# HazyResearch/sampler

Measured on AMD Instinct MI355X. Metric: variables sampled/sec (whole node), higher is better.
Workload: dtype f64 (f32 sampling weights)

## Files before the change

sampler_amd/csrc/dwx_api.cc:

```cpp
#include "../../include/dwx.h"

#include <algorithm>
#include <array>
#include <chrono>
#include <cstdio>
#include <cstdlib>
#include <cmath>
#include <cstring>
#include <map>
#include <memory>
#include <new>
#include <stdexcept>
#include <string>
#include <vector>

#include "device_build.h"
#include "graph_compile.h"
#include "host_parallel.h"
#include "level_build.h"
#if defined(DWX_EMU) && !defined(DWX_EMU_LEVEL_BUILD_UNIT)
#include "level_build.cc"
#endif

#include "sweep_kernels.h"
// ... 64 lines not shown
template <class T>
T *upload_raw(const T *h, size_t n, rt::stream_t s) {
  T *d = (T *)rt::dmalloc(n * sizeof(T));
  rt::h2d(d, h, n * sizeof(T), s);
  return d;
}

struct TimedSpan {
  rt::event_t a, b, c;
  int kind;
  uint32_t launches;
  bool has_pull;
  bool new_sweep;
  uint32_t n_sweeps = 1;
};

template <class... A>
struct Variant {
  void (*fn)(A...) = nullptr;
  size_t lds = 0;
  unsigned cap = 1;
  bool allowed = false;
  void allow() {
    if (!allowed) { rt::allow_dynamic_lds(fn, lds); allowed = true; }
  }
  static Variant eager(void (*f)(A...), size_t bytes) {
    Variant v;
    v.fn = f; v.lds = bytes;
    v.allow();
    v.cap = rt::resident_blocks(f, BLOCK_THREADS, bytes);
    return v;
  }
  Variant lazy(void (*f)(A...)) const {
    Variant v = *this;
    v.fn = f; v.allowed = false;
    return v;
  }
  template <class... B>
  void launch(unsigned grid, unsigned block, rt::stream_t st, B... args) {
    if (!fn) throw std::logic_error("a sweep kernel build that dwx_sampler_create did not resolve for this graph");
    allow();
    rt::launch(fn, grid, block, lds, st, args...);
  }
};
using SweepVariant = Variant<KernelParams>;
using SortedVariant = Variant<KernelParams, const SuperTile *, uint32_t, const SortRec8 *, const double *, uint32_t>;
struct SweepVariants {
  SweepVariant infer[2];
  SweepVariant learn, learn_pull;
  SweepVariant tab[2];
  SweepVariant multi[2][2];
  Variant<KernelParams, MergeArgs> merged[2];
  Variant<KernelParams, PersistArgs> persist;
  SortedVariant sorted_infer[2][2], sorted_learn[2];
};
}

struct dwx_graph {
  std::shared_ptr<CompiledGraph> cg;
};

struct dwx_sampler {
  std::shared_ptr<CompiledGraph> cg;
  dwx_options opts;
  int device = 0;
  rt::stream_t stream = nullptr;
  rt::stream_t side[2] = {nullptr, nullptr};
  rt::event_t ev_fork = nullptr, ev_join[2] = {nullptr, nullptr};
  uint32_t *d_v_meta = nullptr, *d_v_orig = nullptr, *d_v_row = nullptr, *d_v_init = nullptr;
  uint32_t *d_row_ptr = nullptr;
  TileDesc *d_tiles = nullptr;
  uint32_t *d_giant = nullptr, *d_wide = nullptr;
  std::vector<uint32_t> cgiant_tiles, bgiant_tiles, bgiant_piece_off;
  uint32_t *d_bgiant = nullptr, *d_bgiant_piece_off = nullptr, *d_bgiant_decision = nullptr;
  GiantPiece *d_bgiant_pieces = nullptr;
  double *d_bgiant_partial = nullptr;
  int stage_k = 12;
  struct Chunk { uint32_t launch, t0, t1; };
  std::vector<Chunk> plan_chunks;
  uint32_t plan_batches = 1;
  double plan_eta = 0.0;
  bool plan_valid = false;
  std::map<uint32_t, double> row_sum_cache;
  std::vector<uint64_t> sgd_work;
  uint64_t sgd_work_max_launch = 0;
  bool wide_learn = false;
  bool tv_pair = false;
  SweepVariants kv;
  bool rec8 = false;
  bool rp_cat = false;
  bool all_pull = false;
  EdgeRec8 *d_edges8 = nullptr;
  SortRec8 *d_sorted = nullptr;
  SuperTile *d_supers = nullptr;
  double *d_sort_dvals = nullptr;
  uint32_t n_sort_dvals = 0;
  bool sorted_learn = false;
  bool no_sort_uni = false;
  bool sorted_fallback_said = false;
  double *d_row_truth = nullptr, *d_edge_fval64 = nullptr;
  EdgeRec *d_edges = nullptr;
  VifRec *d_vifs = nullptr;
  uint32_t *d_assign_free = nullptr, *d_assign_evid = nullptr, *d_tally = nullptr;
  double *d_weights = nullptr;
  float *d_w32 = nullptr;
  double *d_w_init = nullptr;
  EdgeTerms *d_terms = nullptr;
  int terms_state = 0;
  unsigned long long *d_rb = nullptr;
  bool rb_on = false;
  unsigned long long *d_trace = nullptr;
  uint32_t trace_cap = 0, trace_words = 0, trace_bits = 0;
  uint32_t trace_next = 0, trace_count = 0;
  bool trace_on = false;
  std::vector<uint64_t> trace_ids;
  FactorRec *d_frecs = nullptr;
  VifRec *d_fvifs = nullptr;
  double *d_ffval64 = nullptr;
  uint32_t *d_fwide = nullptr;
  bool score_ready = false;
  bool wstats_ready = false;
  uint64_t wstats_max_count = 0, wstats_max_wid = 0;
  long long *d_pot = nullptr;
  int pot_alloc = 0;
  std::vector<uint8_t> pot_valid;
  bool pot_wanted = false;
  bool last_infer = false;
  bool pot_query_first = false;
  uint64_t pot_supers = 0, pot_sweeps = 0;
  struct Pending {
    bool owed = false;
    bool evid_owed = false;
    uint64_t sweep = 0;
    bool snap = false;
    std::vector<uint8_t> cached;
  } pending;
  bool defer_ok = false;
  float *d_w32_prev = nullptr;
  uint64_t deferred_sweeps = 0, flushes = 0;
  bool has_simple_tiles = false;
  unsigned long long *d_delta = nullptr;
  struct Level {
    std::vector<Chunk> chunks;
    bool fast = false;
    uint32_t *d_inc_wid = nullptr, *d_inc_slot = nullptr;
    float *d_inc_d = nullptr;
    std::vector<uint32_t> inc_begin, inc_end;
    long long *d_t_static = nullptr;
    uint32_t rows = 0;
    double c_max = 0.0, t_max = 0.0;
    std::string range_error;
// ... 161 lines not shown
    rt::event_record(s->ev_fork, s->stream);
    if (any_giant) rt::stream_wait_event(st_giant, s->ev_fork);
    if (any_wide) rt::stream_wait_event(st_wide, s->ev_fork);
  }
  auto launch_lane_tiles = [&](uint32_t a, uint32_t b) {
  if (b <= a) return;
  P.tile_begin = a;
  P.tile_end = b;
  const bool tab8 = s->rec8 && !LEARN && P.edge_terms;
  const bool slim = LEARN && s->rec8 && s->all_pull && !(P.flags & OPT_NO_PULL);
  SweepVariant &k = multi ? kv.multi[rb][trace] : tab8 ? kv.tab[rb] : !LEARN ? kv.infer[rb] : slim ? kv.learn_pull : kv.learn;
  k.launch(std::min<unsigned>(b - a, k.cap), BLOCK_THREADS, s->stream, P);
  ++launches;
  };
  bool used_sorted = false;
  if (s->d_supers && !P.edge_terms && !multi && (!LEARN || (s->sorted_learn && !(P.flags & (OPT_NO_PULL | OPT_DYNAMIC_T))))) {
    const dwx_sampler::Level *lv =
        (LEARN && !P.pot && !default_layout && s->plan_level && s->plan_level->d_supers) ? s->plan_level : nullptr;
    const std::vector<SuperTile> &sv = lv ? lv->sorted_supers : c.supers;
    const SuperTile *d_sv = lv ? lv->d_supers : s->d_supers;
    const SortRec8 *d_sr = lv ? lv->d_sorted : s->d_sorted;
    size_t a = std::lower_bound(sv.begin(), sv.end(), t0, [](const SuperTile &x, uint32_t t) { return x.tile0 < t; }) - sv.begin();
    size_t b = a;
    while (b < sv.size() && sv[b].tile0 + sv[b].ntiles <= t1) ++b;
    struct Run { size_t a, b; };
    std::vector<Run> runs;
    for (size_t i = a; i < b;) {
      size_t j = i + 1;
      while (j < b && sv[j].tile0 == sv[j - 1].tile0 + sv[j - 1].ntiles) ++j;
      runs.push_back({i, j});
      i = j;
    }
    if (runs.size() > 8 && !s->sorted_fallback_said) {
      s->sorted_fallback_said = true;
      fprintf(stderr, "dwx: a launch's weight-sorted super-tiles form %zu gap-free runs (more than 8): its tiles take "
                      "the plain tile sweep (slower weight gathers)\n", runs.size());
    }
    if (!runs.empty() && runs.size() <= 8) {
      used_sorted = true;
      if (covered && sv[runs[0].a].tile0 == t0) *covered = sv[runs[0].b - 1].tile0 + sv[runs[0].b - 1].ntiles;
      uint32_t cursor = t0;
      for (const Run &r : runs) {
        launch_lane_tiles(cursor, sv[r.a].tile0);
        P.super_rot = 0;
        if (LEARN && P.pot) {
          uint32_t n_cached = 0;
          for (size_t i = r.a; i < r.b; ++i)
            if (sv[i].v0 >= P.pot_v0 && sv[i].v0 + sv[i].nv <= P.pot_v1) ++n_cached;
          s->pot_supers += n_cached;
          if (!s->pot_query_first && n_cached < r.b - r.a && sv[r.a].v0 >= P.pot_v0 && sv[r.a].v0 + sv[r.a].nv <= P.pot_v1)
            P.super_rot = n_cached;
        }
        const bool uni = s->n_sort_dvals == 2 && !s->no_sort_uni;
        (LEARN ? kv.sorted_learn[uni] : kv.sorted_infer[uni][rb])
            .launch((unsigned)(r.b - r.a), SORT_THREADS, s->stream, P, (const SuperTile *)(d_sv + r.a), (uint32_t)(r.b - r.a), d_sr,
                    (const double *)s->d_sort_dvals, s->n_sort_dvals);
        ++launches;
        P.super_rot = 0;
        cursor = sv[r.b - 1].tile0 + sv[r.b - 1].ntiles;
      }
      launch_lane_tiles(cursor, t1);
    }
  }
  if (!used_sorted) launch_lane_tiles(t0, t1);
  P.tile_begin = t0;
  P.tile_end = t1;
  if (cg1 > cg0) {
    rt::launch(rb ? giant_kernel<LEARN, RBK> : giant_kernel<LEARN>, cg1 - cg0, GIANT_THREADS, 0, st_giant, P,
               (const uint32_t *)(s->d_giant + cg0), cg1 - cg0);
    ++launches;
  }
  if (bg1 > bg0) {
    const uint32_t p0 = s->bgiant_piece_off[bg0], np = s->bgiant_piece_off[bg1] - p0;
    rt::launch(giant_pot_kernel<LEARN>, np, GIANT_THREADS, 0, st_giant, P, (const uint32_t *)s->d_bgiant,
               (const GiantPiece *)s->d_bgiant_pieces, p0, np, s->d_bgiant_partial);
    rt::launch(rb ? giant_decide_kernel<LEARN, RBK> : giant_decide_kernel<LEARN>, (bg1 - bg0 + BLOCK_THREADS - 1) / BLOCK_THREADS,
               BLOCK_THREADS, 0, st_giant, P, (const uint32_t *)s->d_bgiant, (const uint32_t *)s->d_bgiant_piece_off, bg0, bg1 - bg0,
               (const double *)s->d_bgiant_partial, s->d_bgiant_decision);
    launches += 2;
    if (LEARN) {
      rt::launch(giant_grad_kernel, np, GIANT_THREADS, 0, st_giant, P, (const uint32_t *)s->d_bgiant,
                 (const GiantPiece *)s->d_bgiant_pieces, p0, np, (const uint32_t *)s->d_bgiant_decision);
      ++launches;
    }
  }
  if (w1 > w0) {
    const uint32_t per_block = BLOCK_THREADS / 64u;
    rt::launch(rb ? wide_kernel<LEARN, RBK> : wide_kernel<LEARN>, (w1 - w0 + per_block - 1) / per_block, BLOCK_THREADS, 0,
               st_wide, P, (const uint32_t *)(s->d_wide + w0), w1 - w0);
    ++launches;
  }
  if (fork) {
    if (any_giant) { rt::event_record(s->ev_join[0], st_giant); rt::stream_wait_event(s->stream, s->ev_join[0]); }
    if (any_wide) { rt::event_record(s->ev_join[1], st_wide); rt::stream_wait_event(s->stream, s->ev_join[1]); }
  }
  return launches;
}

bool multi_sweep_graph(const dwx_sampler *s) {
  return s->rec8 && no_binned_tiles(s) && !getenv("DWX_NO_MULTI_SWEEP");
}

void flush_pending(dwx_sampler *s, int chains = 3);
void trace_pack(dwx_sampler *s, uint64_t first_id, uint32_t n_planes, bool unsampled_only) {
  const CompiledGraph &c = *s->cg;
  if (!unsampled_only) flush_pending(s, 2);
  const uint32_t n = (uint32_t)c.Vo;
// ... 877 lines not shown
      t_phase = t;
    };
    s->d_v_meta = upload(c.v_meta, st, 1);
    s->d_v_orig = upload(c.perm, st, 1);
    s->d_v_row = upload(c.v_row, st);
    s->d_v_init = upload(c.v_init, st, 1);
    s->d_row_ptr = upload(c.row_ptr, st, 1);
    {
      std::vector<TileDesc> tiles = c.tiles;
      if (c.ecap > 6 * BLOCK_THREADS) for (auto &t : tiles) t.flags &= ~(TILE_TERMS2 | TILE_TERMS3 | TILE_PULL_UNARY);
      s->d_tiles = upload(tiles, st);
    }
    for (uint32_t ti : c.giant_tiles) ((c.tiles[ti].flags & TILE_CATEGORICAL) ? s->cgiant_tiles : s->bgiant_tiles).push_back(ti);
    s->d_giant = upload(s->cgiant_tiles, st);
    s->d_wide = upload(c.wide_tiles, st);
    {
      std::vector<GiantPiece> pieces;
      s->bgiant_piece_off.assign(1, 0u);
      for (uint32_t slot = 0; slot < s->bgiant_tiles.size(); ++slot) {
        const TileDesc &td = c.tiles[s->bgiant_tiles[slot]];
        for (uint32_t e = td.e0; e < td.e0 + td.nedges; e += GIANT_PIECE)
          pieces.push_back(GiantPiece{slot, e, std::min(e + GIANT_PIECE, td.e0 + td.nedges), 0u});
        if (!td.nedges) pieces.push_back(GiantPiece{slot, td.e0, td.e0, 0u});
        s->bgiant_piece_off.push_back((uint32_t)pieces.size());
      }
      s->d_bgiant = upload(s->bgiant_tiles, st);
      s->d_bgiant_piece_off = upload(s->bgiant_piece_off, st);
      s->d_bgiant_pieces = upload(pieces, st);
      s->d_bgiant_partial = (double *)rt::dmalloc(std::max<size_t>(1, pieces.size()) * 4 * 8);
      rt::dmemset(s->d_bgiant_partial, 0, std::max<size_t>(1, pieces.size()) * 4 * 8, st);
      s->d_bgiant_decision = (uint32_t *)rt::dmalloc(std::max<size_t>(1, s->bgiant_tiles.size()) * 16);
    }
    if (!c.row_truth.empty()) s->d_row_truth = upload(c.row_truth, st);
    if (!c.edge_fval64.empty()) s->d_edge_fval64 = upload(c.edge_fval64, st);
    s->d_edges = upload(c.edges, st, 1);
    s->rec8 = c.edges8.size() != 0;
    if (s->rec8) s->d_edges8 = upload(c.edges8, st, 1);
    s->defer_ok = s->rec8 && !opts->learn_non_evidence && !opts->noise_aware && !getenv("DWX_NO_DEFER");
    if (!c.supers.empty()) {
      s->d_supers = upload(c.supers, st);
      if (c.sorted_deferred) {
        s->d_sorted = (SortRec8 *)rt::dmalloc((c.n_sorted + 1) * sizeof(SortRec8));
        rt::dmemset(s->d_sorted + c.n_sorted, 0, sizeof(SortRec8), st);
        devb::build_sorted_records(s->d_tiles, s->d_edges, s->d_edges8, s->d_supers, (uint32_t)c.supers.size(),
                                   c.sort_dbits.data(), (uint32_t)c.sort_dbits.size(), c.n_sorted, s->d_sorted, (void *)st);
      } else {
        s->d_sorted = upload(c.sorted_recs, st, 1);
      }
      s->d_sort_dvals = upload(c.sort_dvals, st);
      s->n_sort_dvals = (uint32_t)c.sort_dvals.size();
      s->sorted_learn = c.W > LDS_AGG_MAX_W;
      const size_t lds_sorted = sort_lds_bytes(s->n_sort_dvals);
      auto set = [&](SortedVariant &k, auto fn, bool rb) { k.fn = fn; k.lds = lds_sorted; if (!rb) k.allow(); };
      set(s->kv.sorted_infer[0][0], sorted_sweep_kernel<false, false>, false);
      set(s->kv.sorted_infer[0][1], sorted_sweep_kernel<false, false, true>, true);
      set(s->kv.sorted_infer[1][0], sorted_sweep_kernel<false, true>, false);
      set(s->kv.sorted_infer[1][1], sorted_sweep_kernel<false, true, true>, true);
      set(s->kv.sorted_learn[0], sorted_sweep_kernel<true, false>, false);
      set(s->kv.sorted_learn[1], sorted_sweep_kernel<true, true>, false);
      s->no_sort_uni = getenv("DWX_NO_SORT_UNI") != nullptr;
      s->pot_query_first = getenv("DWX_POT_QUERY_FIRST") != nullptr;
    }
    {
      std::vector<VifRec> vifs = c.vifs;
      if (vifs.size() < 4) vifs.resize(4, VifRec{0u, 0u});
      s->d_vifs = upload(vifs, st, 4);
    }
    std::vector<uint32_t> a0(c.V);
    for (uint64_t p = 0; p < c.V; ++p) a0[p] = (c.v_meta[p] & VM_EVIDENCE) ? c.v_init[p] : 0u;
    s->d_assign_free = upload(a0, st);
    s->d_assign_evid = upload(a0, st);
    s->d_tally = (uint32_t *)rt::dmalloc((c.R + 1) * 4);
    rt::dmemset(s->d_tally, 0, (c.R + 1) * 4, st);
    s->d_weights = upload(c.w_init, st);
    phase("upload graph");
    {
      std::vector<float> w32(c.W);
      for (uint64_t i = 0; i < c.W; ++i) w32[i] = (float)c.w_init[i];
      s->d_w32 = upload(w32, st, 1);
      const size_t n_delta = c.tiles.size() * 8 + 2 + (size_t)BP1_TILES * 8;
      s->d_delta = (unsigned long long *)rt::dmalloc(n_delta * 8);
      rt::dmemset(s->d_delta, 0, n_delta * 8, st);
    }
    s->d_w_fixed = upload(c.w_fixed, st);
    s->d_grad = (long long *)rt::dmalloc(c.W * 16);
    rt::dmemset(s->d_grad, 0, c.W * 16, st);

    KernelParams &P = s->base;
    P.v_meta = s->d_v_meta; P.v_orig = s->d_v_orig; P.v_row = s->d_v_row; P.v_init = s->d_v_init;
    P.row_ptr = s->d_row_ptr; P.row_truth = s->d_row_truth; P.edges = s->d_edges; P.edges8 = s->d_edges8; P.edge_terms = nullptr;
    for (const TileDesc &td : c.tiles) if (td.flags & (TILE_SIMPLE | TILE_INLINE2)) { s->has_simple_tiles = true; break; }
    P.edge_fval64 = s->d_edge_fval64; P.vifs = s->d_vifs; P.tiles = s->d_tiles;
    P.assign_free = s->d_assign_free; P.assign_evid = s->d_assign_evid; P.tally = s->d_tally;
    P.w32 = s->d_w32; P.grad = s->d_grad; P.delta = s->d_delta;
    P.seed = opts->seed; P.sweep = 0; P.vid_offset = opts->var_id_offset; P.tile_begin = 0; P.num_weights = (uint32_t)c.W;
    P.flags = (opts->sample_evidence ? OPT_SAMPLE_EVIDENCE : 0) |
              (opts->learn_non_evidence ? OPT_LEARN_NON_EVIDENCE : 0) |
              (opts->noise_aware ? OPT_NOISE_AWARE : 0) |
              (c.has_f64_fval ? OPT_HAS_F64_FVAL : 0) | (c.has_truthiness ? OPT_HAS_TRUTHINESS : 0);
    P.ecap = c.ecap; P.rcap = c.rcap;
    if (c.ecap > MAX_ECAP) throw std::invalid_argument("tile_edges exceeds the staging capacity");
    s->stage_k = c.ecap <= 3 * BLOCK_THREADS ? 3 : (c.ecap <= 6 * BLOCK_THREADS ? 6 : 12);
    const size_t slots = (size_t)s->stage_k * BLOCK_THREADS;
    s->rp_cat = c.edges8.size() != 0 && c.has_categorical && s->stage_k == 6;
    const size_t nrp = std::max<size_t>(c.rcap + 1, (s->rp_cat ? ROWPTR_UNROLL_CAT : ROWPTR_UNROLL) * BLOCK_THREADS);
    size_t off = (nrp * 4 + 15) & ~(size_t)15;
    P.lds_pot_off = c.has_categorical ? (uint32_t)off : 0u;
    if (c.has_categorical) off += (size_t)c.rcap * 8;
    off = (off + 15) & ~(size_t)15;
    P.lds_edge_off = (uint32_t)off;
    s->wide_learn = c.n_terms2_tiles > 0 && s->stage_k <= 6;
    off += slots * sizeof(EdgeRec);
// ... 1275 lines not shown
```

sampler_amd/csrc/sweep_kernels.h:

```cpp
#ifndef DWX_SWEEP_KERNELS_H_
#define DWX_SWEEP_KERNELS_H_

#include <type_traits>

#include "tile_walk.h"

namespace dwx {

DWX_DEV float rec8_signed(uint32_t code, float f) {
  const uint32_t b = float_to_bits(f);
  return bits_to_float(code == 1u ? 0u : (code == 0u ? (b ^ 0x80000000u) : b));
}
DWX_DEV EdgeRec expand_record(const EdgeRec8 &c) {
  EdgeRec r;
  r.wid = c.key & REC8_WID_MASK;
  r.fval = rec8_signed((c.key >> REC8_HIT_SHIFT) & 3u, c.f);
  r.aux = float_to_bits(rec8_signed((c.key >> REC8_MISS_SHIFT) & 3u, c.f));
  r.packed = EDGE_PRESIGNED | (1u << EDGE_ARITY_SHIFT) | ((c.key & REC8_FIXED) ? EDGE_FIXED_FLAG : 0u);
  return r;
}
DWX_DEV EdgeRec expand_record(const EdgeRec &r) { return r; }

template <int K, class Rec = EdgeRec, int RP = (int)ROWPTR_UNROLL>
struct TilePrefetch {
// ... 466 lines not shown
    TileDesc raw_nn = d;
    if (!ONE) {
      raw_nn = P.tiles[has_nn ? nn : tile];
      TileDesc dl = dn;
      if (!has_next) { dl.nedges = 0; dl.nrows = 0; dl.nv = 1; }
      issue_tile_loads<LEARN, K, !TAB>(P, dl, t, f);
    }
    int delta = 0;
    if (MULTI) {
      if (fits) {
        TileView T{s_rowptr, d.r0, s_edges, d.e0, s_w, s_agg, P.lds_pot_off ? s_pot : nullptr};
        const uint32_t n = P.n_sweeps;
        const uint32_t S = (n >= MULTI_SLICE_MIN_SWEEPS && d.nv < BLOCK_THREADS) ? MULTI_SLICES : 1u;
        if (TRACE && P.trace_bits == 1u) {
          infer_bool_multi_trace<W_TERMS, true, RB>(P, T, d.v0 + t, pre, n, t < d.nv);
        } else if (S == 1u) {
          if (t < d.nv) infer_variable_multi<W_TERMS, true, RB, TRACE>(P, T, d.v0 + t, pre, 0u, n, true);
        } else for (uint32_t item = t; item < S * d.nv; item += BLOCK_THREADS) {
          const uint32_t sl = item / d.nv, var = item - sl * d.nv;
          const VarPre vp = var == t ? pre : load_var_pre<false, false>(P, d.v0 + var);
          const uint32_t k_lo = (uint32_t)((uint64_t)n * sl / S), k_hi = (uint32_t)((uint64_t)n * (sl + 1) / S);
          infer_variable_multi<W_TERMS, true, RB, TRACE>(P, T, d.v0 + var, vp, k_lo, k_hi, sl + 1 == S);
        }
      }
    } else if (fits && t < d.nv) {
      TileView T{s_rowptr, d.r0, s_edges, d.e0, s_w, s_agg, P.lds_pot_off ? s_pot : nullptr};
      if (LEARN && pull)
        delta = process_variable<LEARN, W_TERMS8, true, true>(P, T, d.v0 + t, pre, A, B, true);
      else
        process_variable<LEARN, LEARN ? W_ARRAY : (TAB ? W_TERMS8 : W_TERMS), true, true, false, RB>(P, T, d.v0 + t, pre, A, B, false);
    }
    if (pull) {
      const unsigned long long nz = DWX_BALLOT(delta != 0), ng = DWX_BALLOT(delta < 0);
      if ((t & 63u) == 0) {
        unsigned long long *wd = P.delta + ((size_t)tile * 4 + (t >> 6)) * 2;
        DWX_NT_STORE(nz, &wd[0]); DWX_NT_STORE(ng, &wd[1]);
      }
    }
    if (ONE || !has_next) break;
    __syncthreads();
    d = dn;
    dn = scalarise(raw_nn);
    tile = next; next = nn; has_next = has_nn;
  }
  flush_accumulators(P, s_agg, t);
}
template <bool LEARN, int K, bool TAB = false, int RP = (int)ROWPTR_UNROLL, bool MULTI = false, bool RB = false,
          bool TRACE = false>
__global__ void __launch_bounds__(BLOCK_THREADS, TAB ? 4 : (LEARN ? DWX_S8_LEARN_WG : DWX_S8_INFER_WG)) sweep8_kernel(const KernelParams P) {
  sweep8_body<LEARN, K, TAB, RP, MULTI, false, false, RB, TRACE>(P, nullptr);
}


template <bool LEARN, bool UNI = false, bool RB = false>
__global__ void __launch_bounds__(SORT_THREADS, SORT_WG_PER_CU)
sorted_sweep_kernel(const KernelParams P, const SuperTile *supers, uint32_t n_supers, const SortRec8 *recs,
                    const double *dvals, uint32_t n_dvals) {
  DWX_DYN_LDS(dyn_lds);
  uint32_t *s_tv = (uint32_t *)dyn_lds;
  double *s_d = (double *)(dyn_lds + sort_acc_offset(0));
  unsigned long long *s_acc = (unsigned long long *)(dyn_lds + sort_acc_offset(UNI ? 0u : DWX_UNIFORM(n_dvals)));
  const uint32_t t = threadIdx.x;
  if (blockIdx.x >= n_supers) return;
  const uint32_t b = blockIdx.x + P.super_rot;
  SuperTile S = supers[b < n_supers ? b : b - n_supers];
  S.tile0 = DWX_UNIFORM(S.tile0); S.ntiles = DWX_UNIFORM(S.ntiles); S.v0 = DWX_UNIFORM(S.v0); S.nv = DWX_UNIFORM(S.nv);
  S.lo = DWX_UNIFORM(S.lo); S.hi = DWX_UNIFORM(S.hi); S.nrec = DWX_UNIFORM(S.nrec);
  const bool cached = LEARN && P.pot && S.v0 >= P.pot_v0 && S.v0 + S.nv <= P.pot_v1;
  if (cached) S.nrec = 0;
  const SortRec8 *base = recs + (((uint64_t)S.hi << 32) | S.lo);
  SortRec8 rec[SORT_K];
  DWX_LOAD_SORTED_RECORDS(SORT_K, base, S.nrec, 0u, t, rec);
  const double d_uni = UNI ? dvals[1] : 0.0;
  if (!UNI) for (uint32_t i = t; i < n_dvals; i += SORT_THREADS) s_d[i] = dvals[i];
  for (uint32_t i = t; i < S.ntiles; i += SORT_THREADS) s_tv[i] = P.tiles[S.tile0 + i].v0;
  if (t == 0) s_tv[S.ntiles] = S.v0 + S.nv;
  for (uint32_t i = t; i < S.nv; i += SORT_THREADS) s_acc[i] = 0ull;
  __syncthreads();
  constexpr uint32_t STEP = SORT_K * SORT_THREADS;
  for (uint32_t first = 0; first < S.nrec; first += STEP) {
    float w[SORT_K];
#pragma unroll
    for (int k = 0; k < SORT_K; ++k) w[k] = P.w32[rec[k].wid];
    SortRec8 cur[SORT_K];
#pragma unroll
    for (int k = 0; k < SORT_K; ++k) cur[k] = rec[k];
    DWX_LOAD_SORTED_RECORDS(SORT_K, base, S.nrec, first + STEP, t, rec);
#pragma unroll
    for (int k = 0; k < SORT_K; ++k) {
      const uint32_t di = cur[k].od >> SORT_OWNER_BITS;
      const long long q = pot_fix((double)w[k] * (UNI ? d_uni : s_d[di]));
      if (di) atomicAdd(&s_acc[cur[k].od & SORT_OWNER_MASK], (unsigned long long)q);
    }
  }
  constexpr uint32_t TPB = SORT_THREADS / BLOCK_THREADS;
  const uint32_t lane = t & (BLOCK_THREADS - 1), sub = t / BLOCK_THREADS;
  struct Pass { bool have; uint32_t tile, p; bool live; VarPre pre; long long sum; };
  auto issue = [&](uint32_t j0) {
    Pass ps;
    ps.have = j0 + sub < S.ntiles;
    const uint32_t j = ps.have ? j0 + sub : 0u;
    const uint32_t tv0 = s_tv[j], tnv = s_tv[j + 1] - tv0;
    ps.tile = S.tile0 + j;
    ps.live = ps.have && lane < tnv;
    ps.p = tv0 + (lane < tnv ? lane : tnv - 1u);
    ps.pre = load_var_pre<LEARN>(P, ps.p);
    ps.sum = cached ? DWX_NT_LOAD(&P.pot[ps.p]) : 0ll;
    return ps;
  };
  Pass nxt = issue(0u);
  __syncthreads();
  for (uint32_t j0 = 0; j0 < S.ntiles; j0 += TPB) {
    const Pass ps = nxt;
    nxt = issue(j0 + TPB < S.ntiles ? j0 + TPB : j0);
    int delta = 0;
    if (ps.live) {
      double A, B;
      philox_uniforms(P.seed, P.vid_offset + ps.pre.orig, P.sweep, A, B);
      const long long sum = cached ? ps.sum : (long long)s_acc[ps.p - S.v0];
      if (!LEARN && P.pot) DWX_NT_STORE(sum, &P.pot[ps.p]);
      const double x = pot_unfix(sum);
      TileView T{nullptr, 0u, nullptr, 0u, nullptr, nullptr, nullptr};
      T.presum = &x;
      delta = process_variable<LEARN, W_FIXSUM, true, false, false, RB>(P, T, ps.p, ps.pre, A, B, true);
    }
    if (LEARN) {
      const unsigned long long nz = DWX_BALLOT(delta != 0), ng = DWX_BALLOT(delta < 0);
      if (ps.have && (t & 63u) == 0) {
        unsigned long long *wd = P.delta + ((size_t)ps.tile * 4 + (lane >> 6)) * 2;
        DWX_NT_STORE(nz, &wd[0]); DWX_NT_STORE(ng, &wd[1]);
      }
    }
  }
}

template <bool LEARN, bool RB = false>
__global__ void __launch_bounds__(GIANT_THREADS) giant_kernel(const KernelParams P, const uint32_t *giant_tiles,
                                                              uint32_t n) {
  if (blockIdx.x >= n) return;
  const TileDesc d = P.tiles[giant_tiles[blockIdx.x]];
  const uint32_t p = d.v0;
  const VarPre vp = load_var_pre<LEARN>(P, p);
  double A, B;
  philox_uniforms(P.seed, P.vid_offset + vp.orig, P.sweep, A, B);
  const TileView T{P.row_ptr, 0u, P.edges, 0u, nullptr, nullptr, nullptr};
  process_variable<LEARN, W_COOPB, false, false, false, RB>(P, T, p, vp, A, B);
}

struct GiantPiece { uint32_t slot, e0, e1, pad; };

template <bool LEARN>
__global__ void __launch_bounds__(GIANT_THREADS)
giant_pot_kernel(const KernelParams P, const uint32_t *bgiant_tiles, const GiantPiece *pieces, uint32_t piece0,
                 uint32_t n, double *partial) {
  if (blockIdx.x >= n) return;
  const GiantPiece pc = pieces[piece0 + blockIdx.x];
  const uint32_t p = P.tiles[bgiant_tiles[pc.slot]].v0;
  const TileView T{P.row_ptr, 0u, P.edges, 0u, nullptr, nullptr, nullptr};
  double acc[4] = {0.0, 0.0, 0.0, 0.0};
  if (LEARN) {
    const uint32_t *const chains[2] = {P.assign_free, P.assign_evid};
    const int chain[4] = {0, 0, 1, 1};
    const uint32_t prop[4] = {1u, 0u, 1u, 0u};
    const bool hit[4] = {true, false, true, false};
    coop_for_records<W_COOPB, 4, 2>(P, T, pc.e0, pc.e1, p, chains, chain, prop, hit,
                                    [&](const EdgeRec &, uint32_t, double w, const double (&term)[4]) {
#pragma unroll
                                      for (int j = 0; j < 4; ++j) acc[j] += w * term[j];
                                    });
  } else {
    const uint32_t *const chains[1] = {P.assign_evid};
    const int chain[2] = {0, 0};
    const uint32_t prop[2] = {1u, 0u};
    const bool hit[2] = {true, false};
    coop_for_records<W_COOPB, 2, 1>(P, T, pc.e0, pc.e1, p, chains, chain, prop, hit,
                                    [&](const EdgeRec &, uint32_t, double w, const double (&term)[2]) {
                                      acc[2] += w * term[0];
                                      acc[3] += w * term[1];
                                    });
  }
#pragma unroll
  for (int j = LEARN ? 0 : 2; j < 4; ++j) {
    const double v = block_sum_all(acc[j]);
// ... 58 lines not shown
```

sampler_amd/csrc/tile_walk.h:

```cpp
#ifndef DWX_TILE_WALK_H_
#define DWX_TILE_WALK_H_

#include "factor_functions.h"

namespace dwx {

enum { W_GLOBAL = 0, W_ARRAY = 1, W_INRECORD = 2, W_TERMS = 3, W_TERMS8 = 4, W_COOP = 5, W_COOPB = 6, W_PRESUM = 7, W_LREC = 8, W_FIXSUM = 9 };
#ifndef DWX_GIANT_PIECE
#define DWX_GIANT_PIECE 4096
#endif
constexpr uint32_t GIANT_PIECE = DWX_GIANT_PIECE;
#ifndef DWX_GIANT_THREADS
#define DWX_GIANT_THREADS 1024
#endif
constexpr uint32_t GIANT_THREADS = DWX_GIANT_THREADS;
constexpr uint32_t COOP_U = 4;

DWX_DEV uint32_t wave_lane() { return threadIdx.x & 63u; }

DWX_DEV double block_sum_all(double v) {
  __shared__ double s_red[GIANT_THREADS];
  const uint32_t t = threadIdx.x;
  s_red[t] = v;
  __syncthreads();
// ... 691 lines not shown
  if (WMODE == W_LREC) {
    const LearnRec *recs = (const LearnRec *)T.edges;
    const bool evid_hits = evid_value == hit_value, free_hits = free_value == hit_value;
    for (uint32_t e = es; e < ee; ++e) {
      const LearnRec r = recs[e - T.edge_bias];
      if (r.packed & EDGE_FIXED_FLAG) continue;
      const double g = (double)(free_hits ? r.sf1 : r.sf0) - (double)(evid_hits ? r.se1 : r.se0);
      const long long gi = llrint(FIX_SCALE * (t * g));
      const long long ti = count_t ? llrint(FIX_SCALE * t) : 0;
      long long *dst = T.agg ? T.agg : P.grad;
      if (gi) atomicAdd((unsigned long long *)&dst[r.wid], (unsigned long long)gi);
      if (count_t) atomicAdd((unsigned long long *)&dst[P.num_weights + r.wid], (unsigned long long)ti);
    }
    return;
  }
  for (uint32_t e = es; e < ee; ++e) {
    const EdgeRec er = T.edges[e - T.edge_bias];
    if (er.packed & EDGE_FIXED_FLAG) continue;
    double pot_evid, pot_free;
    if (SIMPLE || (er.packed & EDGE_PRESIGNED)) {
      pot_evid = edge_term<true>(P, er, e, P.assign_evid, me, evid_value, evid_value == hit_value);
      pot_free = edge_term<true>(P, er, e, P.assign_free, me, free_value, free_value == hit_value);
    } else {
      const double fv = (er.packed & EDGE_F64_FLAG) ? P.edge_fval64[e] : (double)er.fval;
      const uint32_t prop[2] = {evid_value, free_value};
      double sg[2];
      if (edge_arity(er) == 1u) {
        sg[0] = unary_sign(edge_func(er), prop[0] == er.aux); sg[1] = unary_sign(edge_func(er), prop[1] == er.aux);
      } else {
        const uint32_t *const chains[2] = {P.assign_evid, P.assign_free};
        const int chain[2] = {0, 1};
        record_signs<2, 2>(P, er, me, chains, chain, prop, sg);
      }
      pot_evid = sg[0] * fv;
      pot_free = sg[1] * fv;
    }
    const double g = pot_free - pot_evid;
    const long long gi = llrint(FIX_SCALE * (t * g));
    const long long ti = count_t ? llrint(FIX_SCALE * t) : 0;
    if (T.agg) {
      if (gi) atomicAdd((unsigned long long *)&T.agg[er.wid], (unsigned long long)gi);
      if (count_t) atomicAdd((unsigned long long *)&T.agg[P.num_weights + er.wid], (unsigned long long)ti);
    } else {
      if (gi) atomicAdd((unsigned long long *)&P.grad[er.wid], (unsigned long long)gi);
      if (count_t) atomicAdd((unsigned long long *)&P.grad[P.num_weights + er.wid], (unsigned long long)ti);
    }
  }
}

struct VarPre {
  uint32_t meta, orig, row0, init;
};

template <bool LEARN, bool NT = true>
DWX_DEV VarPre load_var_pre(const KernelParams &P, uint32_t p) {
  VarPre v;
  if (NT) {
    v.meta = DWX_NT_LOAD(&P.v_meta[p]);
    v.orig = DWX_NT_LOAD(&P.v_orig[p]);
    v.row0 = DWX_NT_LOAD(&P.v_row[p]);
    v.init = LEARN ? DWX_NT_LOAD(&P.v_init[p]) : 0u;
  } else {
    v.meta = P.v_meta[p];
    v.orig = P.v_orig[p];
    v.row0 = P.v_row[p];
    v.init = LEARN ? P.v_init[p] : 0u;
  }
  return v;
}

struct TraceCursor {
  uint32_t slot = 0;
  DWX_DEV void init(const KernelParams &P, uint32_t k_lo) {
    const uint32_t k0 = k_lo > P.trace_skip ? k_lo : P.trace_skip;
    slot = (uint32_t)(((uint64_t)P.trace_slot0 + (k0 - P.trace_skip)) % P.trace_cap);
  }
  DWX_DEV unsigned long long *plane(const KernelParams &P) const { return P.trace + (size_t)slot * P.trace_words; }
  DWX_DEV void next(const KernelParams &P) { if (++slot == P.trace_cap) slot = 0; }
};
DWX_DEV void trace_byte(const KernelParams &P, TraceCursor &c, uint32_t k, uint32_t p, uint32_t value) {
  if (k >= P.trace_skip) {
    ((unsigned char *)c.plane(P))[p] = (unsigned char)value;
    c.next(P);
  }
}
template <int WMODE, bool FIXED, bool RB = false, bool TRACE = false>
DWX_DEV void infer_variable_multi(const KernelParams &P, const TileView &T, uint32_t p, const VarPre pre,
                                  const uint32_t k_lo, const uint32_t k_hi, const bool store) {
  const uint32_t meta = pre.meta;
  if ((meta & VM_EVIDENCE) && !(P.flags & OPT_SAMPLE_EVIDENCE)) return;
  const uint32_t card = meta >> VM_CARD_SHIFT, row0 = pre.row0;
  const uint64_t vid = P.vid_offset + pre.orig;
  uint32_t prop = 0;
  TraceCursor tc;
  if (TRACE) tc.init(P, k_lo);
  if (!(meta & VM_CATEGORICAL)) {
    double pp, pn;
    bool_potentials<WMODE, true, FIXED>(P, T, row0, P.assign_evid, p, pp, pn);
    const double scale = 1.0 + exp(pn - pp);
    uint32_t count = 0;
    for (uint32_t k = k_lo; k < k_hi; ++k) {
      double A, B;
      philox_uniforms(P.seed, vid, P.sweep + k, A, B);
      prop = (A * scale < 1.0) ? 1u : 0u;
      count += prop;
      if (TRACE) trace_byte(P, tc, k, p, prop);
    }
    if (count) atomicAdd(&P.tally[row0], count);
    if (RB && k_hi > k_lo) rb_add(P, row0, (unsigned long long)(k_hi - k_lo) * rb_bool_q(pp, pn));
  } else if (card <= SMALL_CARD) {
// ... 46 lines not shown
#pragma unroll
    for (uint32_t d = 0; d < SMALL_CARD; ++d)
      if (d < card && cnt[d]) atomicAdd(&P.tally[row0 + d], cnt[d]);
  } else {
    for (uint32_t k = k_lo; k < k_hi; ++k) {
      double A, B;
      philox_uniforms(P.seed, vid, P.sweep + k, A, B);
      prop = cat_draw<WMODE, true, RB>(P, T, row0, card, P.assign_evid, p, A);
      atomicAdd(&P.tally[row0 + prop], 1u);
      if (TRACE) trace_byte(P, tc, k, p, prop);
    }
  }
  if (store) DWX_NT_STORE(prop, &P.assign_evid[p]);
}

template <int WMODE, bool FIXED, bool RB>
DWX_DEV void infer_bool_multi_trace(const KernelParams &P, const TileView &T, uint32_t p, const VarPre pre,
                                    const uint32_t n, const bool in_tile) {
  const bool active = in_tile && !((pre.meta & VM_EVIDENCE) && !(P.flags & OPT_SAMPLE_EVIDENCE));
  const uint32_t row0 = pre.row0;
  const uint64_t vid = P.vid_offset + pre.orig;
  double pp = 0.0, pn = 0.0;
  if (active) bool_potentials<WMODE, true, FIXED>(P, T, row0, P.assign_evid, p, pp, pn);
  const double scale = 1.0 + exp(pn - pp);
  const uint32_t lane = threadIdx.x & 63u, p0 = p - lane;
  const uint32_t sh = p0 & 63u;
  const size_t w = p0 >> 6;
  TraceCursor tc;
  tc.init(P, 0u);
  uint32_t prop = 0, count = 0;
  for (uint32_t k = 0; k < n; ++k) {
    if (active) {
      double A, B;
      philox_uniforms(P.seed, vid, P.sweep + k, A, B);
      prop = (A * scale < 1.0) ? 1u : 0u;
      count += prop;
    }
    const unsigned long long m = DWX_BALLOT(active && prop);
    if (k >= P.trace_skip) {
      if (lane == 0 && m) {
        unsigned long long *plane = tc.plane(P);
        atomicAdd(&plane[w], m << sh);
        if (sh && (m >> (64u - sh))) atomicAdd(&plane[w + 1], m >> (64u - sh));
      }
      tc.next(P);
    }
  }
  if (!active) return;
  if (count) atomicAdd(&P.tally[row0], count);
  if (RB && n) rb_add(P, row0, (unsigned long long)n * rb_bool_q(pp, pn));
  DWX_NT_STORE(prop, &P.assign_evid[p]);
}

template <bool LEARN, int WMODE, bool SIMPLE, bool FIXED = false, bool NOCAT = false, bool RB = false>
DWX_DEV int process_variable(const KernelParams &P, const TileView &T, uint32_t p,
                             const VarPre pre, double A, double B, const bool want_delta = false) {
  const uint32_t meta = pre.meta;
  const bool is_cat = !NOCAT && (meta & VM_CATEGORICAL);
  const bool is_evid = meta & VM_EVIDENCE;
  const uint32_t card = meta >> VM_CARD_SHIFT;
  const uint32_t row0 = pre.row0;
  static_assert(!(LEARN && RB), "Rao-Blackwellised sums: inference sweeps only");
  constexpr bool COOP = Coop<WMODE>::on;
  const bool leader = !COOP || Coop<WMODE>::lane() == 0u;
  if (!LEARN) {
    if (is_evid && !(P.flags & OPT_SAMPLE_EVIDENCE)) return 0;
    uint32_t prop;
    if (!is_cat) {
      double pp, pn;
      bool_potentials<WMODE, SIMPLE, FIXED>(P, T, row0, P.assign_evid, p, pp, pn);
      prop = bool_draw(A, pp, pn);
      if (prop && leader) atomicAdd(&P.tally[row0], 1u);
      if (RB && leader) rb_add_owner(P, row0, rb_bool_q(pp, pn));
    } else {
      prop = cat_draw<WMODE, SIMPLE, RB>(P, T, row0, card, P.assign_evid, p, A);
      if (leader) atomicAdd(&P.tally[row0 + prop], 1u);
    }
    if (SIMPLE) DWX_NT_STORE(prop, &P.assign_evid[p]); else if (leader) P.assign_evid[p] = prop;
    return 0;
  }
  const bool noise_aware = P.flags & OPT_NOISE_AWARE;
  const bool has_truth = meta & VM_TRUTHINESS;
  uint32_t p_free;
  double pp_f = 0.0, pn_f = 0.0;
  const bool both = !SIMPLE && !is_cat && !(!noise_aware && is_evid) && !(noise_aware && has_truth);
  double pp_e = 0.0, pn_e = 0.0;
  if (!is_cat) {
    if (both) bool_potentials_both<WMODE>(P, T, row0, p, pp_f, pn_f, pp_e, pn_e);
    else bool_potentials<WMODE, SIMPLE, FIXED>(P, T, row0, P.assign_free, p, pp_f, pn_f);
    p_free = bool_draw(A, pp_f, pn_f);
  } else {
    p_free = cat_draw<WMODE, SIMPLE>(P, T, row0, card, P.assign_free, p, A);
  }
  if (SIMPLE) DWX_NT_STORE(p_free, &P.assign_free[p]); else if (leader) P.assign_free[p] = p_free;
  const uint32_t evid_value = pre.init;
  uint32_t p_evid;
  if (!noise_aware && is_evid) {
    p_evid = evid_value;
  } else if (noise_aware && has_truth) {
    double sum = 0;
    p_evid = 0;
    for (uint32_t i = 0; i < card; ++i) {
      sum += P.row_truth[row0 + i];
      if (sum >= B) { p_evid = i; break; }
    }
  } else if (!is_cat) {
    const double pp = SIMPLE ? pp_f : pp_e, pn = SIMPLE ? pn_f : pn_e;
    p_evid = bool_draw(B, pp, pn);
  } else {
    p_evid = cat_draw<WMODE, SIMPLE>(P, T, row0, card, P.assign_evid, p, B);
  }
  if (!(P.flags & OPT_FREE_CHAIN_ONLY)) {
    if (SIMPLE) DWX_NT_STORE(p_evid, &P.assign_evid[p]); else if (leader) P.assign_evid[p] = p_evid;
  }
  if (!(P.flags & OPT_LEARN_NON_EVIDENCE) &&
      ((!noise_aware && !is_evid) || (noise_aware && !has_truth)))
    return 0;
  if (!is_cat) {
    const bool dyn_t = P.flags & OPT_DYNAMIC_T;
    if (SIMPLE && !dyn_t && p_free == evid_value) return 0;
    if (SIMPLE && want_delta) return (int)p_free - (int)evid_value;
    sgd_row<SIMPLE, WMODE>(P, T, row0, p, evid_value, p_free, 1u, 1.0, dyn_t);
    return 0;
  }
  for (uint32_t val = 0; val < card; ++val) {
    if (!noise_aware && val != evid_value) continue;
    double t = 1.0;
    if (noise_aware) {
      t = P.row_truth ? P.row_truth[row0 + val] : 0.0;
      if (is_linear_zero(t)) continue;
    }
    sgd_row<SIMPLE, WMODE>(P, T, row0 + val, p, val, p_free, val, t, true);
    if (val == p_free) continue;
    sgd_row<SIMPLE, WMODE>(P, T, row0 + p_free, p, val, p_free, p_free, t, true);
  }
  return 0;
}


DWX_DEV uint32_t compress_even_bits(unsigned long long x) {
  x &= 0x5555555555555555ull;
  x = (x | (x >> 1)) & 0x3333333333333333ull;
  x = (x | (x >> 2)) & 0x0F0F0F0F0F0F0F0Full;
  x = (x | (x >> 4)) & 0x00FF00FF00FF00FFull;
  x = (x | (x >> 8)) & 0x0000FFFF0000FFFFull;
  x = (x | (x >> 16)) & 0x00000000FFFFFFFFull;
  return (uint32_t)x;
}

template <class Rec>
DWX_DEV int learn_variable_terms2(const KernelParams &P, const uint32_t *rowptr, uint32_t row_bias,
                                  const Rec *recs, uint32_t edge_bias, long long *agg,
                                  uint32_t p, const VarPre pre, double A, double B, const bool pull_unary) {
  const bool is_evid = pre.meta & VM_EVIDENCE;
  const bool noise_aware = P.flags & OPT_NOISE_AWARE;
  const uint32_t es = rowptr[pre.row0 - row_bias], ee = rowptr[pre.row0 + 1 - row_bias];
  double ppf = 0.0, pnf = 0.0, ppe = 0.0, pne = 0.0;
  for (uint32_t e = es; e < ee; e += LEARN_BATCH) {
    Rec r[LEARN_BATCH];
#pragma unroll
    for (uint32_t u = 0; u < LEARN_BATCH; ++u) r[u] = recs[umin(e + u, ee - 1) - edge_bias];
#pragma unroll
    for (uint32_t u = 0; u < LEARN_BATCH; ++u) {
      const bool in = e + u < ee;
      const double w = (double)r[u].w;
      ppf += in ? w * (double)lrec_term(r[u], 0u, 1u) : 0.0; pnf += in ? w * (double)lrec_term(r[u], 0u, 0u) : 0.0;
      ppe += in ? w * (double)lrec_term(r[u], 1u, 1u) : 0.0; pne += in ? w * (double)lrec_term(r[u], 1u, 0u) : 0.0;
    }
  }
  const uint32_t p_free = bool_draw(A, ppf, pnf);
// ... 83 lines not shown
```

Before: 55.95 billion.

## Add plain sorted-sweep builds with batched prefetch of per-variable words

Adds PLAIN specialisations of the sorted sweep kernel for runs without noise-aware, learn-non-evidence or sample-evidence options. In the query-only inference range these skip loading the meta and init words, and in learning they skip the row word, which trims per-variable memory traffic and branches. The loop now prefetches variable metadata for several passes at once (SORT_DRAW_BATCH, default 4) instead of one, so more loads are in flight. This raises register pressure and depends on the query-tile range check staying correct. The PLAIN learning path also returns the delta directly, without the DYNAMIC_T check.

```diff
diff --git a/sampler_amd/csrc/dwx_api.cc b/sampler_amd/csrc/dwx_api.cc
--- a/sampler_amd/csrc/dwx_api.cc
+++ b/sampler_amd/csrc/dwx_api.cc
@@ -140,7 +140,7 @@
   SweepVariant multi[2][2];
   Variant<KernelParams, MergeArgs> merged[2];
   Variant<KernelParams, PersistArgs> persist;
-  SortedVariant sorted_infer[2][2], sorted_learn[2];
+  SortedVariant sorted_infer[2][2][2], sorted_learn[2][2];
 };
 }
 
@@ -185,6 +185,7 @@
   uint32_t n_sort_dvals = 0;
   bool sorted_learn = false;
   bool no_sort_uni = false;
+  bool sort_plain = false;
   bool sorted_fallback_said = false;
   double *d_row_truth = nullptr, *d_edge_fval64 = nullptr;
   EdgeRec *d_edges = nullptr;
@@ -452,7 +453,8 @@
             P.super_rot = n_cached;
         }
         const bool uni = s->n_sort_dvals == 2 && !s->no_sort_uni;
-        (LEARN ? kv.sorted_learn[uni] : kv.sorted_infer[uni][rb])
+        const bool plain = s->sort_plain && (LEARN || (!rb && t1 <= c.launch_query_tile_end[l]));
+        (LEARN ? kv.sorted_learn[uni][plain] : kv.sorted_infer[uni][rb][plain])
             .launch((unsigned)(r.b - r.a), SORT_THREADS, s->stream, P, (const SuperTile *)(d_sv + r.a), (uint32_t)(r.b - r.a), d_sr,
                     (const double *)s->d_sort_dvals, s->n_sort_dvals);
         ++launches;
@@ -1436,12 +1438,19 @@
       s->sorted_learn = c.W > LDS_AGG_MAX_W;
       const size_t lds_sorted = sort_lds_bytes(s->n_sort_dvals);
       auto set = [&](SortedVariant &k, auto fn, bool rb) { k.fn = fn; k.lds = lds_sorted; if (!rb) k.allow(); };
-      set(s->kv.sorted_infer[0][0], sorted_sweep_kernel<false, false>, false);
-      set(s->kv.sorted_infer[0][1], sorted_sweep_kernel<false, false, true>, true);
-      set(s->kv.sorted_infer[1][0], sorted_sweep_kernel<false, true>, false);
-      set(s->kv.sorted_infer[1][1], sorted_sweep_kernel<false, true, true>, true);
-      set(s->kv.sorted_learn[0], sorted_sweep_kernel<true, false>, false);
-      set(s->kv.sorted_learn[1], sorted_sweep_kernel<true, true>, false);
+      set(s->kv.sorted_infer[0][0][0], sorted_sweep_kernel<false, false>, false);
+      set(s->kv.sorted_infer[0][1][0], sorted_sweep_kernel<false, false, true>, true);
+      set(s->kv.sorted_infer[1][0][0], sorted_sweep_kernel<false, true>, false);
+      set(s->kv.sorted_infer[1][1][0], sorted_sweep_kernel<false, true, true>, true);
+      set(s->kv.sorted_learn[0][0], sorted_sweep_kernel<true, false>, false);
+      set(s->kv.sorted_learn[1][0], sorted_sweep_kernel<true, true>, false);
+      s->sort_plain = !opts->noise_aware && !opts->learn_non_evidence && !opts->sample_evidence && !getenv("DWX_NO_SORT_PLAIN");
+      if (s->sort_plain) {
+        set(s->kv.sorted_infer[0][0][1], sorted_sweep_kernel<false, false, false, true>, false);
+        set(s->kv.sorted_infer[1][0][1], sorted_sweep_kernel<false, true, false, true>, false);
+        set(s->kv.sorted_learn[0][1], sorted_sweep_kernel<true, false, false, true>, false);
+        set(s->kv.sorted_learn[1][1], sorted_sweep_kernel<true, true, false, true>, false);
+      }
       s->no_sort_uni = getenv("DWX_NO_SORT_UNI") != nullptr;
       s->pot_query_first = getenv("DWX_POT_QUERY_FIRST") != nullptr;
     }
diff --git a/sampler_amd/csrc/sweep_kernels.h b/sampler_amd/csrc/sweep_kernels.h
--- a/sampler_amd/csrc/sweep_kernels.h
+++ b/sampler_amd/csrc/sweep_kernels.h
@@ -542,7 +542,12 @@
 }
 
 
-template <bool LEARN, bool UNI = false, bool RB = false>
+#ifndef DWX_SORT_DRAW_BATCH
+#define DWX_SORT_DRAW_BATCH 4
+#endif
+constexpr uint32_t SORT_DRAW_BATCH = DWX_SORT_DRAW_BATCH;
+static_assert(SORT_DRAW_BATCH >= 1 && SORT_DRAW_BATCH <= 16, "passes per batch of sorted_sweep_kernel's draws");
+template <bool LEARN, bool UNI = false, bool RB = false, bool PLAIN = false>
 __global__ void __launch_bounds__(SORT_THREADS, SORT_WG_PER_CU)
 sorted_sweep_kernel(const KernelParams P, const SuperTile *supers, uint32_t n_supers, const SortRec8 *recs,
                     const double *dvals, uint32_t n_dvals) {
@@ -583,42 +588,59 @@
       if (di) atomicAdd(&s_acc[cur[k].od & SORT_OWNER_MASK], (unsigned long long)q);
     }
   }
-  constexpr uint32_t TPB = SORT_THREADS / BLOCK_THREADS;
+  constexpr uint32_t TPB = SORT_THREADS / BLOCK_THREADS, U = SORT_DRAW_BATCH, BT = U * TPB;
   const uint32_t lane = t & (BLOCK_THREADS - 1), sub = t / BLOCK_THREADS;
-  struct Pass { bool have; uint32_t tile, p; bool live; VarPre pre; long long sum; };
-  auto issue = [&](uint32_t j0) {
-    Pass ps;
-    ps.have = j0 + sub < S.ntiles;
-    const uint32_t j = ps.have ? j0 + sub : 0u;
+  struct Where { bool have, live; uint32_t tile, p; };
+  auto where = [&](uint32_t j0) {
+    Where w;
+    w.have = j0 + sub < S.ntiles;
+    const uint32_t j = w.have ? j0 + sub : 0u;
     const uint32_t tv0 = s_tv[j], tnv = s_tv[j + 1] - tv0;
-    ps.tile = S.tile0 + j;
-    ps.live = ps.have && lane < tnv;
-    ps.p = tv0 + (lane < tnv ? lane : tnv - 1u);
-    ps.pre = load_var_pre<LEARN>(P, ps.p);
-    ps.sum = cached ? DWX_NT_LOAD(&P.pot[ps.p]) : 0ll;
-    return ps;
+    w.tile = S.tile0 + j;
+    w.live = w.have && lane < tnv;
+    w.p = tv0 + (lane < tnv ? lane : tnv - 1u);
+    return w;
   };
-  Pass nxt = issue(0u);
+  struct Pass { VarPre pre; long long sum; };
+  auto issue = [&](uint32_t jb, Pass (&ps)[U]) {
+#pragma unroll
+    for (uint32_t u = 0; u < U; ++u) {
+      const uint32_t p = where(jb + u * TPB).p;
+      ps[u].pre = load_var_pre<LEARN, true, PLAIN>(P, p);
+      ps[u].sum = cached ? DWX_NT_LOAD(&P.pot[p]) : 0ll;
+    }
+  };
+  Pass nxt[U];
+  issue(0u, nxt);
   __syncthreads();
-  for (uint32_t j0 = 0; j0 < S.ntiles; j0 += TPB) {
-    const Pass ps = nxt;
-    nxt = issue(j0 + TPB < S.ntiles ? j0 + TPB : j0);
-    int delta = 0;
-    if (ps.live) {
-      double A, B;
-      philox_uniforms(P.seed, P.vid_offset + ps.pre.orig, P.sweep, A, B);
-      const long long sum = cached ? ps.sum : (long long)s_acc[ps.p - S.v0];
-      if (!LEARN && P.pot) DWX_NT_STORE(sum, &P.pot[ps.p]);
-      const double x = pot_unfix(sum);
-      TileView T{nullptr, 0u, nullptr, 0u, nullptr, nullptr, nullptr};
-      T.presum = &x;
-      delta = process_variable<LEARN, W_FIXSUM, true, false, false, RB>(P, T, ps.p, ps.pre, A, B, true);
-    }
-    if (LEARN) {
-      const unsigned long long nz = DWX_BALLOT(delta != 0), ng = DWX_BALLOT(delta < 0);
-      if (ps.have && (t & 63u) == 0) {
-        unsigned long long *wd = P.delta + ((size_t)ps.tile * 4 + (lane >> 6)) * 2;
-        DWX_NT_STORE(nz, &wd[0]); DWX_NT_STORE(ng, &wd[1]);
+  for (uint32_t jb = 0; jb < S.ntiles; jb += BT) {
+    Pass cur[U];
+#pragma unroll
+    for (uint32_t u = 0; u < U; ++u) cur[u] = nxt[u];
+    issue(jb + BT < S.ntiles ? jb + BT : jb, nxt);
+#pragma unroll
+    for (uint32_t u = 0; u < U; ++u) {
+      const uint32_t j0 = jb + u * TPB;
+      if (u && j0 >= S.ntiles) break;
+      const Where w = where(j0);
+      const Pass ps = cur[u];
+      int delta = 0;
+      if (w.live) {
+        double A, B;
+        philox_uniforms(P.seed, P.vid_offset + ps.pre.orig, P.sweep, A, B);
+        const long long sum = cached ? ps.sum : (long long)s_acc[w.p - S.v0];
+        if (!LEARN && P.pot) DWX_NT_STORE(sum, &P.pot[w.p]);
+        const double x = pot_unfix(sum);
+        TileView T{nullptr, 0u, nullptr, 0u, nullptr, nullptr, nullptr};
+        T.presum = &x;
+        delta = process_variable<LEARN, W_FIXSUM, true, false, true, RB, PLAIN>(P, T, w.p, ps.pre, A, B, true);
+      }
+      if (LEARN) {
+        const unsigned long long nz = DWX_BALLOT(delta != 0), ng = DWX_BALLOT(delta < 0);
+        if (w.have && (t & 63u) == 0) {
+          unsigned long long *wd = P.delta + ((size_t)w.tile * 4 + (lane >> 6)) * 2;
+          DWX_NT_STORE(nz, &wd[0]); DWX_NT_STORE(ng, &wd[1]);
+        }
       }
     }
   }
diff --git a/sampler_amd/csrc/tile_walk.h b/sampler_amd/csrc/tile_walk.h
--- a/sampler_amd/csrc/tile_walk.h
+++ b/sampler_amd/csrc/tile_walk.h
@@ -767,10 +767,16 @@
   uint32_t meta, orig, row0, init;
 };
 
-template <bool LEARN, bool NT = true>
+template <bool LEARN, bool NT = true, bool PLAIN = false>
 DWX_DEV VarPre load_var_pre(const KernelParams &P, uint32_t p) {
   VarPre v;
-  if (NT) {
+  if (PLAIN) {
+    static_assert(!PLAIN || NT, "the plain builds stream their words");
+    v.meta = LEARN ? DWX_NT_LOAD(&P.v_meta[p]) : 0u;
+    v.orig = DWX_NT_LOAD(&P.v_orig[p]);
+    v.row0 = LEARN ? 0u : DWX_NT_LOAD(&P.v_row[p]);
+    v.init = LEARN ? DWX_NT_LOAD(&P.v_init[p]) : 0u;
+  } else if (NT) {
     v.meta = DWX_NT_LOAD(&P.v_meta[p]);
     v.orig = DWX_NT_LOAD(&P.v_orig[p]);
     v.row0 = DWX_NT_LOAD(&P.v_row[p]);
@@ -923,19 +929,20 @@
   DWX_NT_STORE(prop, &P.assign_evid[p]);
 }
 
-template <bool LEARN, int WMODE, bool SIMPLE, bool FIXED = false, bool NOCAT = false, bool RB = false>
+template <bool LEARN, int WMODE, bool SIMPLE, bool FIXED = false, bool NOCAT = false, bool RB = false, bool PLAIN = false>
 DWX_DEV int process_variable(const KernelParams &P, const TileView &T, uint32_t p,
                              const VarPre pre, double A, double B, const bool want_delta = false) {
+  static_assert(!PLAIN || (SIMPLE && NOCAT && !RB && WMODE == W_FIXSUM), "the plain builds: sorted_sweep_kernel's");
   const uint32_t meta = pre.meta;
   const bool is_cat = !NOCAT && (meta & VM_CATEGORICAL);
-  const bool is_evid = meta & VM_EVIDENCE;
+  const bool is_evid = (LEARN || !PLAIN) && (meta & VM_EVIDENCE);
   const uint32_t card = meta >> VM_CARD_SHIFT;
   const uint32_t row0 = pre.row0;
   static_assert(!(LEARN && RB), "Rao-Blackwellised sums: inference sweeps only");
   constexpr bool COOP = Coop<WMODE>::on;
   const bool leader = !COOP || Coop<WMODE>::lane() == 0u;
   if (!LEARN) {
-    if (is_evid && !(P.flags & OPT_SAMPLE_EVIDENCE)) return 0;
+    if (!PLAIN && is_evid && !(P.flags & OPT_SAMPLE_EVIDENCE)) return 0;
     uint32_t prop;
     if (!is_cat) {
       double pp, pn;
@@ -950,7 +957,7 @@
     if (SIMPLE) DWX_NT_STORE(prop, &P.assign_evid[p]); else if (leader) P.assign_evid[p] = prop;
     return 0;
   }
-  const bool noise_aware = P.flags & OPT_NOISE_AWARE;
+  const bool noise_aware = !PLAIN && (P.flags & OPT_NOISE_AWARE);
   const bool has_truth = meta & VM_TRUTHINESS;
   uint32_t p_free;
   double pp_f = 0.0, pn_f = 0.0;
@@ -984,9 +991,10 @@
   if (!(P.flags & OPT_FREE_CHAIN_ONLY)) {
     if (SIMPLE) DWX_NT_STORE(p_evid, &P.assign_evid[p]); else if (leader) P.assign_evid[p] = p_evid;
   }
-  if (!(P.flags & OPT_LEARN_NON_EVIDENCE) &&
+  if ((PLAIN || !(P.flags & OPT_LEARN_NON_EVIDENCE)) &&
       ((!noise_aware && !is_evid) || (noise_aware && !has_truth)))
     return 0;
+  if (PLAIN) return (int)p_free - (int)evid_value;
   if (!is_cat) {
     const bool dyn_t = P.flags & OPT_DYNAMIC_T;
     if (SIMPLE && !dyn_t && p_free == evid_value) return 0;
```

Measured after the change: 55.87 billion. Within noise of the previous version (-0.1%).
